# transferia/transferia

Hardware: AMD Instinct MI355X
Metric: ChangeItems/sec through CSV parse -> mask(ClientIP)+filter(EventDate) -> devnull, ClickBench hits, HBM-resident input (the PCIe-inclusive rate is `pcie_inclusive`) (higher is better)
Workload: dtype u8; 1 GPU; ClickBench hits-1M CSV parse -> mask(ip)+filter(EventDate) -> devnull (BASELINE.json configs[1]); columns=105, parallelism=row-range shard x1, no collective, rows_per_pass=1048576, csv_bytes_per_pass=838371857

## Files before the change

### transferia_amd/csrc/tf_common.hpp

```cpp
#pragma once
#include <hip/hip_runtime.h>

#include <cstdint>
#include <cstdio>
#include <cstring>
#include <memory>
#include <mutex>
#include <unordered_map>
#include <stdexcept>
#include <string>
#include <vector>

#include "../../include/tfgpu.h"

#ifndef TF_DYNAMIC_LDS
#define TF_DYNAMIC_LDS(type, name) extern __shared__ type name[]
#endif

#ifndef TF_GLOBAL_PTR
#define TF_GLOBAL_PTR(T, p) ((T *)(__attribute__((address_space(1))) T *)(p))
#endif

#ifndef TF_LOAD16_STREAM
__device__ __forceinline__ uint4 tf_load16_stream(const void *p) {
// ... 122 lines not shown
struct PinScope { PinScope() {} };
void d2h(void *dst, const void *src, size_t n);
void d2d(void *dst, const void *src, size_t n);
void sync();

inline bool repr_is_var(int r) { return r == TFGPU_R_STRING || r == TFGPU_R_BYTES || r == TFGPU_R_JSONNUM || r == TFGPU_R_JSON; }
inline size_t repr_width(int r) {
  switch (r) {
    case TFGPU_R_INT8: case TFGPU_R_UINT8: case TFGPU_R_BOOL: return 1;
    case TFGPU_R_INT16: case TFGPU_R_UINT16: return 2;
    case TFGPU_R_INT32: case TFGPU_R_UINT32: case TFGPU_R_FLOAT32: return 4;
    case TFGPU_R_INT64: case TFGPU_R_UINT64: case TFGPU_R_FLOAT64: case TFGPU_R_TIME: case TFGPU_R_DURATION: return 8;
    default: return 0;
  }
}

struct TextView {
  Buf src;
  Buf fstart;
  uint8_t quote = '"';
  bool jsonnum = false;
  bool has_special = true;
  Buf packed;
};
struct DColumn {
  std::string name;
  int dtype = TFGPU_T_INVALID;
  int repr = TFGPU_R_INVALID;
  Buf values, offsets, data, nanos, validity;
  Buf absent;
  uint64_t data_len = 0;
  std::shared_ptr<TextView> view;
  const Buf &payload() const { return (!data && view) ? view->packed : data; }
  bool lazy() const { return !data && view && !view->packed; }
};
void materialize(const struct ::tfgpu_dbatch &b, const std::vector<const DColumn *> *only = nullptr);
void dense(const struct ::tfgpu_dbatch *b, bool absent_ok = false);
void dense_locked(const struct ::tfgpu_dbatch &b);
int lanes_created();
uint64_t lane_generation();
std::unique_ptr<struct ::tfgpu_dbatch> snapshot(const struct ::tfgpu_dbatch &b);
bool has_absent(const struct ::tfgpu_dbatch &b);
Buf validity_minus_absent(const Buf &validity, const Buf &absent, int64_t nrows);
Buf find_device_block(const void *p);
void register_device_block(const Buf &b);

}

namespace tf {
struct PendingRows {
  std::shared_ptr<const struct ::tfgpu_dbatch> src;
  Buf sel;
};
}

struct tfgpu_dbatch {
  int64_t nrows = 0;
  std::vector<tf::DColumn> cols;
  std::shared_ptr<tf::PendingRows> pending;
// ... 4 lines not shown
  std::vector<std::pair<std::string, int>> schema;
  std::vector<std::string> key_names;
  std::vector<tf::DColumn> old_keys;
  tf::Buf old_present;
  std::string ns, table;
  tf::Buf kind, src_row, part_id;
  tf::Buf col_order;
};

struct tfgpu_dbuf {
  tf::Buf mem;
  uint64_t size = 0;
};

namespace tf {
inline std::unique_ptr<tfgpu_dbatch> shallow_copy(const tfgpu_dbatch &in) { return std::make_unique<tfgpu_dbatch>(in); }
template <class F> void materialize_where(const tfgpu_dbatch &b, F pred) {
  std::vector<const DColumn *> need;
  for (auto &c : b.cols) if (pred(c)) need.push_back(&c);
  materialize(b, &need);
}
void exclusive_scan_u32(const uint32_t *in, uint32_t *out, int64_t n, bool with_total);
void exclusive_scan_u32_segments(uint32_t *inout, int64_t seg_len, int nseg, int64_t seg_stride);
bool select_kept_u32(const uint32_t *keep, int64_t n, int32_t *sel, uint32_t *count);
const uint32_t *any_nonzero_to_host(const uint32_t *v, int64_t n);
const uint32_t *segment_totals_to_host(const uint32_t *scanned, int64_t seg_len, int nseg, int64_t seg_stride);
void sum_u32_segments_u64(const uint32_t *in, int64_t seg_len, int nseg, int64_t seg_stride, unsigned long long *totals);

}
```

### transferia_amd/csrc/tf_csv.hip

```cpp
#include <algorithm>
#include <cmath>
#include <cstdio>
#include <type_traits>

#include "tf_devfmt.hpp"
#include "tf_devparse.hpp"
#include "tf_devfloat.hpp"
#include "tf_segcopy.hpp"
#include "tf_textview.hpp"
#include "tf_wave.hpp"
#include "tf_swar.hpp"
#include "tf_gotime.hpp"
#include "tf_f64range.hpp"
#include "tf_plan.hpp"
#include "tf_strictcell.hpp"

#ifdef TF_CSV_ABLATE_BUILD
#define CSV_ABL(x) ((x).ablate)
#else
#define CSV_ABL(x) 0
#endif
namespace tf {

std::unique_ptr<tfgpu_dbatch> compact_rows(const tfgpu_dbatch &in, Buf keep);
// ... 1657 lines not shown

__global__ void csv_collect(const uint32_t *nerr, const uint32_t *last, const uint32_t *lens_all, int64_t seg_stride, int64_t nrows, int nstr, const uint32_t *fstart_all,
                            int64_t fstride, uint32_t *out, const uint32_t *spec, int64_t ntiles, int64_t skip, const uint32_t *lines_total, const uint32_t *ovf) {
  int i = threadIdx.x;
  if (ovf) {
    const uint32_t nl = *lines_total;
    if (i == 2) { out[2 + 2 * nstr] = nl; out[3 + 2 * nstr] = *ovf; }
    nrows = min(nrows, max((int64_t)nl - skip, (int64_t)0));
    if (i == 1) out[1] = *last;
  } else if (spec) {
    const uint32_t nl = ntiles ? (spec[2 + ntiles - 1] & SP_VAL) : 0u;
    if (i == 2) { out[2 + 2 * nstr] = nl; out[3 + 2 * nstr] = spec[1]; }
    nrows = min(nrows, max((int64_t)nl - skip, (int64_t)0));
    uint32_t le = 0;
    for (int64_t hi = ntiles - 1; hi >= 0 && le == 0; hi -= 64) {
      const int64_t t = hi - i;
      const uint32_t v = t >= 0 ? spec[2 + ntiles + t] : 0u;
      const uint64_t has = __ballot(v != 0);
      if (has) le = (uint32_t)__shfl((int)v, __ffsll((long long)has) - 1, 64);
    }
    if (i == 1) out[1] = le;
  } else if (i == 1) out[1] = *last;
  if (i == 0) out[0] = *nerr;
  for (int s = i; s < nstr; s += blockDim.x) { out[2 + s] = lens_all[(int64_t)s * seg_stride + nrows]; out[2 + nstr + s] = fstart_all[(int64_t)s * fstride + FS_HDR - 1]; }
}
__global__ void csv_zero_flags(uint32_t *fstart_all, int64_t fstride, int nstr, uint32_t *slow, uint32_t *gen, uint32_t *nerr, uint32_t *ovf) {
  for (int s = threadIdx.x; s < nstr; s += blockDim.x) fstart_all[(int64_t)s * fstride + FS_HDR - 1] = 0;
  if (threadIdx.x < 2) { slow[threadIdx.x] = 0; gen[threadIdx.x] = 0; }
  if (threadIdx.x == 2) *nerr = 0;
  if (threadIdx.x == 3 && ovf) *ovf = 0;
}
__global__ void csv_keep_from_err(const uint8_t *err, int64_t n, uint32_t *keep) {
  int64_t r = (int64_t)blockIdx.x * blockDim.x + threadIdx.x;
  if (r < n) keep[r] = err[r] ? 0u : 1u;
}

__global__ void csv_shift_rows(const uint32_t *row_start, int64_t n, uint32_t *out) {
  int64_t i = (int64_t)blockIdx.x * blockDim.x + threadIdx.x;
  if (i <= n) out[i] = row_start[i];
}

__global__ void __launch_bounds__(256) csv_ml_line_fn(const uint8_t *data, const uint32_t *row_start, int64_t nlines, uint8_t quote, uint8_t escape, uint8_t *fn) {
  const int64_t i = (int64_t)blockIdx.x * blockDim.x + threadIdx.x;
  if (i >= nlines) return;
  const uint64_t a = row_start[i], b = row_start[i + 1];
  if (b - a <= 1) { fn[i] = 2u | 4u; return; }
  MemBytes m(data);
// ... 86 lines not shown

uint32_t newline_starts(const uint8_t *data, uint64_t len, Buf *out) {
  hipStream_t st = ctx().stream;
  const int64_t ntiles = (int64_t)((len + NL_TILE - 1) / NL_TILE), ngran = (int64_t)((len + CSV_GRAN - 1) / CSV_GRAN);
  uint32_t n = 0;
  Buf tile_counts = dalloc((size_t)(ngran + 1) * 4);
  if (ntiles) {
    { KernelTimer t("csv_count_newlines"); csv_count_newlines<<<(unsigned)ntiles, NL_THREADS, 0, st>>>(data, len, ptr<uint32_t>(tile_counts), ngran); }
    exclusive_scan_u32(ptr<uint32_t>(tile_counts), ptr<uint32_t>(tile_counts), ngran, true);
    const uint32_t *h = d2h_u32(ptr<uint32_t>(tile_counts) + ngran);
    tf::sync();
    n = *h;
  }
  *out = dalloc_zero((size_t)(n + 2) * 4);
  if (n) { KernelTimer t("csv_line_index"); csv_line_index<<<(unsigned)ntiles, NL_THREADS, 0, st>>>(data, len, ptr<uint32_t>(tile_counts), ptr<uint32_t>(*out)); }
  return n;
}

static void materialize_cols(const tfgpu_dbatch &b, const std::vector<const DColumn *> *only, const uint8_t *text) {
  hipStream_t st = ctx().stream;
  const int64_t nrows = b.nrows;
  struct Grp { const uint8_t *src; uint8_t quote; std::vector<CopyCol> all, lng, sht; };
  std::vector<Grp> groups;
  auto visit = [&](const DColumn &d) {
    if (!d.lazy()) return;
    if (only && std::find(only->begin(), only->end(), &d) == only->end()) return;
    TextView &v = *d.view;
    const uint8_t *src = text ? text : ptr<uint8_t>(v.src);
    if (!src) throw Error(TFGPU_ERR_INVALID, "internal: text column " + d.name + " lost its source text");
    v.packed = dalloc(d.data_len + 8);
    CopyCol c{ptr<uint32_t>(d.offsets), ptr<uint32_t>(v.fstart), ptr<uint8_t>(v.packed), v.jsonnum ? 1 : 0, nullptr, 0};
    Grp *g = nullptr;
    for (auto &x : groups) if (x.src == src && x.quote == v.quote) g = &x;
    if (!g) { groups.push_back(Grp{src, v.quote, {}, {}, {}}); g = &groups.back(); }
    if (v.has_special) g->all.push_back(c);
    ((d.data_len >= (uint64_t)nrows * 8) ? g->lng : g->sht).push_back(c);
  };
  for (auto &d : b.cols) visit(d);
  for (auto &d : b.old_keys) visit(d);
  if (!nrows) return;
  for (auto &g : groups) {
    Buf ball = upload_small(g.all.data(), g.all.size() * sizeof(CopyCol));
    Buf blng = upload_small(g.lng.data(), g.lng.size() * sizeof(CopyCol)), bsht = upload_small(g.sht.data(), g.sht.size() * sizeof(CopyCol));
    KernelTimer t("csv_copy_words");
    if (!g.lng.empty()) { CopyParams cp{g.src, nrows, ptr<CopyCol>(blng), (int32_t)g.lng.size(), g.quote}; csv_copy_words<1><<<dim3((unsigned)((nrows + 255) / 256), (unsigned)g.lng.size()), 256, 0, st>>>(cp); }
    if (!g.sht.empty()) { CopyParams cp{g.src, nrows, ptr<CopyCol>(bsht), (int32_t)g.sht.size(), g.quote}; csv_copy_cells<<<dim3((unsigned)((nrows + 255) / 256), (unsigned)((g.sht.size() + CC_GROUP - 1) / CC_GROUP)), 256, 0, st>>>(cp); }
// ... 432 lines not shown
  if (ablate) {
    TF_HIP(hipMemsetAsync(lens_all->p, 0, (size_t)std::max(nstr, 1) * (size_t)seg_stride * 4, st));
    TF_HIP(hipMemsetAsync(fstart_all->p, 0, (size_t)std::max(nstr, 1) * (size_t)fstride * 4, st));
    TF_HIP(hipMemsetAsync(err->p, 0, (size_t)nrows + 16, st));
    for (auto &d : db->cols) { if (d.values) TF_HIP(hipMemsetAsync(d.values->p, 0, d.values->bytes, st)); if (d.nanos) TF_HIP(hipMemsetAsync(d.nanos->p, 0, d.nanos->bytes, st)); }
  }
  if (nrows && rowpath) {
    KernelTimer t("csv_parse_rows");
    csv_parse_rows<<<blocks_for(nrows, 256), 256, 0, st>>>(pp);
  } else if (nlines) {
    if (use_lanes) {
      const int64_t per_xcd = (ltiles + 7) / 8;
      KernelTimer t("csv_parse_lanes");
      csv_parse_lanes<<<(unsigned)(per_xcd * 8), CL_THREADS, 0, st>>>(pp);
    } else {
      const int64_t per_xcd = (rtiles + 7) / 8;
      KernelTimer t("csv_parse_regular");
      if (pp.col_lanes) csv_parse_cols<<<(unsigned)(spec ? rtiles : per_xcd * 8), CT_THREADS, 0, st>>>(pp);
      else csv_parse_regular<<<(unsigned)(spec ? rtiles : per_xcd * 8), CT_THREADS, 0, st>>>(pp);
    }
    { KernelTimer t("csv_parse_tiles_general"); csv_parse_tiles_general<<<(unsigned)std::min<int64_t>(ntiles + rtiles, 2048), CT_THREADS, 0, st>>>(pp); }
    { KernelTimer t("csv_parse_listed"); csv_parse_listed<<<(unsigned)std::min<int64_t>(blocks_for(slow_cap, 64), 1024), 64, 0, st>>>(pp); }
  }
  if (nrows && nstr) {
    csv_zero_err_lens<<<blocks_for(nrows, 256), 256, 0, st>>>(ptr<uint8_t>(err), nrows, ptr<CsvCol>(bcols), ncols, ahead ? ptr<uint32_t>(tile_counts) + ngran : nullptr, skip);
    exclusive_scan_u32_segments(ptr<uint32_t>(lens_all), nrows, nstr, seg_stride);
  } else if (nstr) {
    TF_HIP(hipMemsetAsync(lens_all->p, 0, (size_t)nstr * (size_t)seg_stride * 4, st));
  }
  Buf summary = dalloc((size_t)(2 * nstr + 4) * 4);
  csv_collect<<<1, 64, 0, st>>>(ptr<uint32_t>(nerr), rowpath ? ptr<uint32_t>(row_start) + nlines : pp.last_end, ptr<uint32_t>(lens_all),
                                seg_stride, nrows, nstr, ptr<uint32_t>(fstart_all), fstride, ptr<uint32_t>(summary), pp.spec, rtiles, skip,
                                ptr<uint32_t>(tile_counts) + (spec ? 0 : ngran), pp.ovf);
  const uint32_t *hsum = d2h_u32(summary->p, (size_t)(2 * nstr) + 4);
  tf::sync();
  const uint32_t hnerr = hsum[0], last = hsum[1];
  if (spec || ahead) {
    const uint32_t nl_true = hsum[2 + 2 * nstr], overflow = hsum[3 + 2 * nstr];
    if (overflow || nl_true > cap_lines || (int64_t)nl_true < skip || (nl_true && !last)) { *retry = true; return TFGPU_OK; }
    nlines = nl_true; nlogical = nl_true; nrows = (int64_t)nl_true - skip;
    db->nrows = nrows;
  }
  if (!rowpath && nlines >= 16 && last) { cx.csv_hint_bpl = (double)last / (double)nlines; cx.csv_hint_ncols = schema->ncols; }
  if (phases && !rowpath) {
    unsigned long long ph[8]; d2h(ph, bphase->p, sizeof ph); tf::sync();
    std::fprintf(stderr, "tfgpu csv phases (s_memtime ticks per workgroup, %lld tiles): stage %.0f classify %.0f fields %.0f index %.0f cells(wave 0) %.0f cells-barrier %.0f epilogue %.0f\n", (long long)rtiles,
                 (double)ph[0] / rtiles, (double)ph[1] / rtiles, (double)ph[2] / rtiles, (double)ph[3] / rtiles, (double)ph[4] / rtiles, (double)ph[5] / rtiles, (double)ph[6] / rtiles);
  }
  static const bool debug = [] { const char *e = std::getenv("TFGPU_CSV_DEBUG"); return e && e[0] == '1'; }();
  if (debug && !rowpath) {
    uint32_t g = 0, sl = 0;
    d2h(&g, gen->p, 4); d2h(&sl, slow->p, 4);
    tf::sync();
    std::fprintf(stderr, "tfgpu csv: %s, %lld tiles of %u KiB, %u general pieces; %u lines, %u per-row\n", use_lanes ? "lanes" : "regular", (long long)(use_lanes ? ltiles : rtiles), (use_lanes ? cl_tile(pp.tile_cpt) : tile_bytes) / 1024u, g, nlines, sl);
  }

  Buf src_block = staged ? staged : find_device_block(data);
  static const bool force_eager = [] { const char *e = std::getenv("TFGPU_CSV_EAGER"); return e && e[0] == '1'; }();
  for (int s = 0; s < nstr; s++) {
    DColumn &d = db->cols[(size_t)str_col_index[(size_t)s]];
    d.data_len = hsum[2 + s];
    d.offsets = subbuf(lens_all, (size_t)s * (size_t)seg_stride * 4, (size_t)(nrows + 1) * 4);
    if (rowpath) continue;
    auto v = std::make_shared<TextView>();
    v->src = src_block ? src_block : nullptr;
    v->fstart = subbuf(fstart_all, ((size_t)s * (size_t)fstride + FS_HDR) * 4, (size_t)std::max<int64_t>(nrows, 1) * 4);
    v->has_special = hsum[2 + nstr + s] != 0;
    v->quote = opts->quote_char; v->jsonnum = d.repr == TFGPU_R_JSONNUM;
    d.view = std::move(v);
  }
  if (nstr && rowpath) {
    std::vector<CopyCol> cc;
    for (int s = 0; s < nstr; s++) {
      DColumn &d = db->cols[(size_t)str_col_index[(size_t)s]];
      d.data = dalloc(d.data_len + 8);
      const CsvCol &hc = cols[(size_t)str_col_index[(size_t)s]];
      cc.push_back(CopyCol{ptr<uint32_t>(d.offsets), hc.fstart, ptr<uint8_t>(d.data), d.repr == TFGPU_R_JSONNUM ? 1 : 0, hc.patch, dp.empty() ? 0u : (uint32_t)dp.size()});
    }
    Buf bcc = up(cc.data(), cc.size() * sizeof(CopyCol));
    if (nrows) {
      CopyParams cp{data, nrows, ptr<CopyCol>(bcc), nstr, opts->quote_char};
      KernelTimer t("csv_copy_strings");
      csv_copy_strings<<<blocks_for(nrows, 256), 256, 0, st>>>(cp);
    }
  } else if (nstr && (!src_block || force_eager)) {
    materialize_from(*db, data);
  }

  for (int i : sys_cols) {
    std::string detail;
    const int rc = fill_system_column(db->cols[(size_t)i], nrows, opts->file_name, opts->row_number_base, nullptr, opts->hide_system_cols, &detail);
// ... 40 lines not shown
```

### transferia_amd/csrc/tf_devcol.hpp

```cpp
#pragma once
#include "tf_common.hpp"

namespace tf {

struct DCol {
  const void *values;
  const uint32_t *offsets;
  const uint8_t *data;
  const int32_t *nanos;
  const uint8_t *validity;
  int32_t repr;
  int32_t dtype;
};
static inline DCol dcol_of(const DColumn &c) {
  DCol d;
  d.values = c.values ? c.values->p : nullptr;
  d.offsets = ptr<uint32_t>(c.offsets);
  if (c.lazy()) throw Error(TFGPU_ERR_INVALID, "internal: text column " + c.name + " read before materialize()");
  d.data = ptr<uint8_t>(c.payload());
  d.nanos = ptr<int32_t>(c.nanos);
  d.validity = ptr<uint8_t>(c.validity);
  d.repr = c.repr; d.dtype = c.dtype;
  return d;
}
__device__ __forceinline__ bool is_valid(const DCol &c, int64_t r) { return !c.validity || ((c.validity[r >> 3] >> (r & 7)) & 1); }


}
```

### transferia_amd/csrc/tf_mask.hip

```cpp
#include "tf_plan.hpp"
#include "tf_rows.hpp"
#include "tf_devrow.hpp"
#include "tf_emit.hpp"

namespace tf {
__constant__ uint32_t SHA_K[64] = {
    0x428a2f98, 0x71374491, 0xb5c0fbcf, 0xe9b5dba5, 0x3956c25b, 0x59f111f1, 0x923f82a4, 0xab1c5ed5, 0xd807aa98, 0x12835b01, 0x243185be,
    0x550c7dc3, 0x72be5d74, 0x80deb1fe, 0x9bdc06a7, 0xc19bf174, 0xe49b69c1, 0xefbe4786, 0x0fc19dc6, 0x240ca1cc, 0x2de92c6f, 0x4a7484aa,
    0x5cb0a9dc, 0x76f988da, 0x983e5152, 0xa831c66d, 0xb00327c8, 0xbf597fc7, 0xc6e00bf3, 0xd5a79147, 0x06ca6351, 0x14292967, 0x27b70a85,
    0x2e1b2138, 0x4d2c6dfc, 0x53380d13, 0x650a7354, 0x766a0abb, 0x81c2c92e, 0x92722c85, 0xa2bfe8a1, 0xa81a664b, 0xc24b8b70, 0xc76c51a3,
    0xd192e819, 0xd6990624, 0xf40e3585, 0x106aa070, 0x19a4c116, 0x1e376c08, 0x2748774c, 0x34b0bcb5, 0x391c0cb3, 0x4ed8aa4a, 0x5b9cca4f,
    0x682e6ff3, 0x748f82ee, 0x78a5636f, 0x84c87814, 0x8cc70208, 0x90befffa, 0xa4506ceb, 0xbef9a3f7, 0xc67178f2};

__device__ __forceinline__ uint32_t rotr32(uint32_t x, int n) { return __builtin_rotateright32(x, n); }

__device__ __forceinline__ void sha256_compress(uint32_t st[8], uint32_t w[16]) {
  uint32_t a = st[0], b = st[1], c = st[2], d = st[3], e = st[4], f = st[5], g = st[6], h = st[7];
#pragma unroll
  for (int i = 0; i < 64; i++) {
    if (i >= 16) {
      uint32_t w15 = w[(i - 15) & 15], w2 = w[(i - 2) & 15];
      uint32_t s0 = rotr32(w15, 7) ^ rotr32(w15, 18) ^ (w15 >> 3);
      uint32_t s1 = rotr32(w2, 17) ^ rotr32(w2, 19) ^ (w2 >> 10);
      w[i & 15] = w[i & 15] + s0 + w[(i - 7) & 15] + s1;
// ... 101 lines not shown
      uint32_t n0 = (half >> 12) & 15, n1 = (half >> 8) & 15, n2 = (half >> 4) & 15, n3 = half & 15;
      auto hx = [](uint32_t n) { return n + (n < 10 ? '0' : 'a' - 10); };
      o[k] = hx(n0) | hx(n1) << 8 | hx(n2) << 16 | hx(n3) << 24;
    }
    dst[q] = make_uint4(o[0], o[1], o[2], o[3]);
  }
  p.offsets[ro] = (uint32_t)(ro * 64);
  if (ro == p.nrows - 1) p.offsets[p.nrows] = (uint32_t)(p.nrows * 64);
}


void mask_precheck(const tfgpu_plan &p, const tfgpu_dbatch &in) {
  for (auto &c : (in.pending ? in.pending->src->cols : in.cols)) {
    if (!p.mask_has(c.name)) continue;
    bool done = false;
    for (auto &r : in.replaced) if (r.name == c.name) done = true;
    if (done) continue;
    require_serializable(c, "mask_field");
    if ((uint64_t)in.nrows * 64 > 0xFFFFFFFFull) throw Error(TFGPU_ERR_UNSUPPORTED, "mask_field: batch too large for 32-bit offsets; split the batch by rows");
  }
}

std::unique_ptr<tfgpu_dbatch> apply_mask(const tfgpu_plan &p, const tfgpu_dbatch &in) {
  auto out = shallow_copy(in);
  for (auto &sc : out->schema) if (p.mask_has(sc.first)) sc.second = TFGPU_T_UTF8;
  hipStream_t st = ctx().stream;
  const tfgpu_dbatch &from = in.pending ? *in.pending->src : in;
  const int32_t *sel = in.pending ? ptr<int32_t>(in.pending->sel) : nullptr;
  auto replaced_at = [&](const std::string &name) -> int { for (size_t i = 0; i < in.replaced.size(); i++) if (in.replaced[i].name == name) return (int)i; return -1; };
  materialize_where(from, [&](const DColumn &c) { return p.mask_has(c.name) && replaced_at(c.name) < 0; });
  const int64_t n = in.nrows;
  auto mask_one = [&](const DColumn &c, const int32_t *through) {
    require_serializable(c, "mask_field");
    if ((uint64_t)n * 64 > 0xFFFFFFFFull) throw Error(TFGPU_ERR_UNSUPPORTED, "mask_field: batch too large for 32-bit offsets; split the batch by rows");
    DColumn o;
    o.name = c.name; o.dtype = TFGPU_T_UTF8; o.repr = TFGPU_R_STRING;
    o.data_len = (uint64_t)n * 64;
    o.data = dalloc(o.data_len);
    o.offsets = dalloc((size_t)(n + 1) * 4);
    MaskParams mp;
    mp.col = dcol_of(c);
    std::memcpy(mp.ipad, p.ipad_state, sizeof mp.ipad);
    std::memcpy(mp.opad, p.opad_state, sizeof mp.opad);
    mp.nrows = n; mp.out = ptr<uint8_t>(o.data); mp.offsets = ptr<uint32_t>(o.offsets); mp.sel = through;
    {
      KernelTimer t("mask_hmac_sha256", n);
      if (n) mask_hmac_kernel<<<grid_for(n, 256), 256, 0, st>>>(mp);
    }
    if (!n) TF_HIP(hipMemsetAsync(o.offsets->p, 0, 4, st));
    return o;
  };
  if (!in.pending) {
    for (auto &c : out->cols) if (p.mask_has(c.name)) {
// ... 16 lines not shown
```

### transferia_amd/csrc/tf_rows.hip

```cpp
#include <chrono>
#include <thread>

#include "tf_rows.hpp"
#include "tf_devrow.hpp"
#include "tf_segcopy.hpp"
#include "tf_textview.hpp"

namespace tf {
__global__ void __launch_bounds__(256) build_selection_kernel(const uint32_t *__restrict__ keep_scan, int64_t n, int32_t *__restrict__ sel) {
  int64_t i = (int64_t)blockIdx.x * blockDim.x + threadIdx.x;
  if (i >= n) return;
  uint32_t a = keep_scan[i], b = keep_scan[i + 1];
  if (a != b) sel[a] = (int32_t)i;
}

struct GFix { const void *in; void *out; int32_t width; int32_t pad; };
template <class T> __device__ __forceinline__ void gather_run(const GFix *__restrict__ a, int lo, int hi, int32_t s, int64_t k) {
  constexpr int U = 8;
  int i = lo;
  for (; i + U <= hi; i += U) {
    T v[U];
#pragma unroll
    for (int q = 0; q < U; q++) v[q] = TF_GLOBAL_PTR(const T, a[i + q].in)[s];
#pragma unroll
// ... 73 lines not shown
    if (n) { fsv = g.fstart[sel[k]]; if (cell_plain(fsv)) n = 0; }
  }
  text_copy_special_wave(g.in_data, g.quote, g.out_data, g.jsonnum != 0, fsv, o0, n, threadIdx.x & 63);
}
__global__ void collect_totals(const uint32_t *lens_all, int64_t seg_stride, int64_t m, int nv, uint32_t *out) {
  for (int s = threadIdx.x; s < nv; s += blockDim.x) out[s] = lens_all[(int64_t)s * seg_stride + m];
}

static std::unique_ptr<tfgpu_dbatch> gather_batch(const tfgpu_dbatch &in, const Buf &sel, int64_t m, const std::vector<DColumn> *skip = nullptr) {
  if (in.col_order) throw Error(TFGPU_ERR_UNSUPPORTED, "the batch's rows carry their own ColumnNames order (tfgpu_batch.col_order: a collapsed TOAST batch); row-moving steps do not carry it — "
                                                       "view / download, the native queue format and the Debezium emitter read it");
  auto out = std::make_unique<tfgpu_dbatch>();
  out->nrows = m; out->ns = in.ns; out->table = in.table; out->schema = in.schema;
  hipStream_t st = ctx().stream;
  const int32_t *sp = ptr<int32_t>(sel);
  unsigned g = grid_for(m, 256);
  KernelTimer t("compact_gather");
  static const bool eager_text = [] { const char *e = std::getenv("TFGPU_CSV_EAGER"); return e && e[0] == '1'; }();
  std::vector<GFix> fx; std::vector<GVar> vr; std::vector<size_t> var_cols; std::vector<GBit> bits;
  const size_t ncur = in.cols.size(), nall = ncur + in.old_keys.size();
  auto col_at = [&](size_t i) -> const DColumn & { return i < ncur ? in.cols[i] : in.old_keys[i - ncur]; };
  out->cols.reserve(ncur); out->old_keys.reserve(in.old_keys.size());
  out->key_names = in.key_names;
  int nvar = 0;
  for (size_t i = 0; i < nall; i++) if (repr_is_var(col_at(i).repr) && !(skip && i < ncur && [&] { for (auto &r : *skip) if (r.name == in.cols[i].name) return true; return false; }())) nvar++;
  const int64_t seg_stride = ((m + 1 + 3) / 4) * 4;
  Buf lens_all = nvar ? dalloc((size_t)nvar * (size_t)seg_stride * 4 + 16) : nullptr;
  auto skipped = [&](size_t ai) -> const DColumn * {
    if (!skip || ai >= ncur) return nullptr;
    for (auto &r : *skip) if (r.name == in.cols[ai].name) return &r;
    return nullptr;
  };
  for (size_t ai = 0; ai < nall; ai++) {
    const DColumn &c = col_at(ai);
    if (const DColumn *have = skipped(ai)) { out->cols.push_back(*have); continue; }
    DColumn o;
    o.name = c.name; o.dtype = c.dtype; o.repr = c.repr;
    if (repr_is_var(c.repr)) {
      size_t si = vr.size();
      o.offsets = subbuf(lens_all, si * (size_t)seg_stride * 4, (size_t)(m + 1) * 4);
      if (!c.lazy() || eager_text) o.data = dalloc(c.data_len + 8);
      o.data_len = c.data_len;
      if (c.lazy() && !eager_text) {
        if (!c.view->src) throw Error(TFGPU_ERR_INVALID, "internal: text column " + c.name + " lost its source text");
        auto v = std::make_shared<TextView>();
        v->src = c.view->src; v->fstart = dalloc((size_t)std::max<int64_t>(m, 1) * 4);
        v->has_special = c.view->has_special; v->quote = c.view->quote; v->jsonnum = c.view->jsonnum;
        fx.push_back(GFix{c.view->fstart->p, v->fstart->p, 4, 0});
        o.view = std::move(v);
        o.data = nullptr;
        vr.push_back(GVar{ptr<uint32_t>(c.offsets), nullptr, ptr<uint32_t>(o.offsets), nullptr, nullptr, 0, 0, 0});
      } else if (c.lazy()) {
        if (!c.view->src) throw Error(TFGPU_ERR_INVALID, "internal: text column " + c.name + " lost its source text");
        vr.push_back(GVar{ptr<uint32_t>(c.offsets), ptr<uint8_t>(c.view->src), ptr<uint32_t>(o.offsets), ptr<uint8_t>(o.data), ptr<uint32_t>(c.view->fstart), c.view->quote, c.view->jsonnum ? 1u : 0u, c.view->has_special ? 1u : 0u});
      } else vr.push_back(GVar{ptr<uint32_t>(c.offsets), ptr<uint8_t>(c.payload()), ptr<uint32_t>(o.offsets), ptr<uint8_t>(o.data), nullptr, 0, 0, 0});
      var_cols.push_back(ai);
    } else {
      size_t w = repr_width(c.repr);
      o.values = dalloc((size_t)m * w);
      fx.push_back(GFix{c.values->p, o.values->p, (int32_t)w, 0});
      if (c.nanos) { o.nanos = dalloc((size_t)m * 4); fx.push_back(GFix{c.nanos->p, o.nanos->p, 4, 0}); }
// ... 27 lines not shown
    exclusive_scan_u32_segments(ptr<uint32_t>(lens_all), m, nvar, seg_stride);
    if (m) {
      std::vector<GVar> lng, sht;
      for (size_t i = 0; i < vr.size(); i++) if (vr[i].out_data) ((col_at(var_cols[i]).data_len >= (uint64_t)in.nrows * 8) ? lng : sht).push_back(vr[i]);
      Buf blng = upload_const(lng.data(), lng.size() * sizeof(GVar)), bsht = upload_const(sht.data(), sht.size() * sizeof(GVar));
      if (!lng.empty()) gather_bytes_all<1><<<dim3(grid_for(m, 256), (unsigned)lng.size()), 256, 0, st>>>(ptr<GVar>(blng), sp, m);
      if (!sht.empty()) gather_bytes_cells<<<dim3(grid_for(m, 256), (unsigned)sht.size()), 256, 0, st>>>(ptr<GVar>(bsht), sp, m);
      std::vector<GVar> lz;
      for (auto &x : vr) if (x.fstart && x.has_special) lz.push_back(x);
      if (!lz.empty()) {
        Buf blz = upload_const(lz.data(), lz.size() * sizeof(GVar));
        gather_text_special<<<dim3(grid_for(m, 256), (unsigned)lz.size()), 256, 0, st>>>(ptr<GVar>(blz), sp, m);
      }
    }
    Buf tot = dalloc((size_t)nvar * 4);
    collect_totals<<<1, 64, 0, st>>>(ptr<uint32_t>(lens_all), seg_stride, m, nvar, ptr<uint32_t>(tot));
    const uint32_t *h = d2h_u32(tot->p, (size_t)nvar);
    sync();
    for (int i = 0; i < nvar; i++) out_at(var_cols[(size_t)i]).data_len = h[i];
  }
  return out;
}

std::unique_ptr<tfgpu_dbatch> gather_rows(const tfgpu_dbatch &in, const Buf &sel, int64_t m) { return gather_batch(in, sel, m); }

static bool lazy_rows_on() {
  static const bool off = [] { const char *e = std::getenv("TFGPU_LAZY_ROWS"); return e && e[0] == '0'; }();
  return !off;
}
std::unique_ptr<tfgpu_dbatch> compact(const tfgpu_dbatch &in, Buf keep , bool lazy) {
  int64_t n = in.nrows;
  Buf sel = dalloc((size_t)n * 4 + 4);
  const uint32_t *hm;
  if (select_kept_u32(ptr<uint32_t>(keep), n, ptr<int32_t>(sel), ptr<uint32_t>(keep) + n)) hm = d2h_u32(ptr<uint32_t>(keep) + n);
  else {
    exclusive_scan_u32(ptr<uint32_t>(keep), ptr<uint32_t>(keep), n, true);
    hm = d2h_u32(ptr<uint32_t>(keep) + n);
    if (n) build_selection_kernel<<<grid_for(n, 256), 256, 0, ctx().stream>>>(ptr<uint32_t>(keep), n, ptr<int32_t>(sel));
  }
  sync();
  const uint32_t m = *hm;
  if ((int64_t)m == n) return shallow_copy(in);
  if (lazy && lazy_rows_on() && !in.pending && m) {
    auto out = std::make_unique<tfgpu_dbatch>();
    out->nrows = m; out->ns = in.ns; out->table = in.table; out->schema = in.schema; out->key_names = in.key_names;
    auto pr = std::make_shared<PendingRows>();
// ... 96 lines not shown
```

### transferia_amd/csrc/tf_scan.hip

```cpp
#include "tf_common.hpp"
#include "tf_wave.hpp"

namespace tf {

static constexpr int SCAN_THREADS = 256;
static constexpr int SCAN_WAVES = SCAN_THREADS / 64;
static constexpr int SCAN_ITEMS = 16;
static constexpr int SCAN_TILE = SCAN_THREADS * SCAN_ITEMS;
static constexpr int64_t RAW_SUMS_MAX = 1024;

__device__ __forceinline__ void scan_load16(const uint32_t *__restrict__ src, int64_t base, int64_t n, bool fast, uint32_t v[SCAN_ITEMS]) {
  if (fast) {
    const uint4 *p = reinterpret_cast<const uint4 *>(src + base);
#pragma unroll
    for (int i = 0; i < SCAN_ITEMS / 4; i++) { uint4 q = p[i]; v[4 * i] = q.x; v[4 * i + 1] = q.y; v[4 * i + 2] = q.z; v[4 * i + 3] = q.w; }
  } else {
#pragma unroll
    for (int i = 0; i < SCAN_ITEMS; i++) v[i] = (base + i < n) ? src[base + i] : 0;
  }
}

__global__ void __launch_bounds__(SCAN_THREADS) scan_reduce_kernel(const uint32_t *__restrict__ in, uint32_t *__restrict__ sums,
                                                                  int64_t n, int64_t seg_stride, int64_t nblocks) {
  __shared__ uint32_t lds[SCAN_WAVES];
// ... 121 lines not shown
}

__global__ void __launch_bounds__(256) any_nonzero_kernel(const uint32_t *v, int64_t n, uint32_t *flag) {
  bool hit = false;
  for (int64_t i = (int64_t)blockIdx.x * 256 + threadIdx.x; i < n; i += (int64_t)gridDim.x * 256) hit |= v[i] != 0;
  if (__ballot(hit) && (threadIdx.x & 63) == 0) atomicOr(flag, 1u);
}
const uint32_t *any_nonzero_to_host(const uint32_t *v, int64_t n) {
  Buf flag = dalloc_zero(4);
  if (n > 0) any_nonzero_kernel<<<(unsigned)std::min<int64_t>((n + 255) / 256, 1024), 256, 0, ctx().stream>>>(v, n, ptr<uint32_t>(flag));
  return d2h_u32(flag->p, 1);
}

void exclusive_scan_u32(const uint32_t *in, uint32_t *out, int64_t n, bool with_total) {
  KernelTimer t("scan_u32");
  scan_impl(in, out, n, 0, 1, with_total);
}

void exclusive_scan_u32_segments(uint32_t *inout, int64_t seg_len, int nseg, int64_t seg_stride) {
  if (nseg <= 0) return;
  KernelTimer t("scan_u32_segments");
  scan_impl(inout, inout, seg_len, seg_stride, nseg, true);
}

}
```

### transferia_amd/csrc/tf_sizeof.hip

```cpp
#include "tf_devcol.hpp"
#include "tf_wave.hpp"

using namespace tf;

namespace {

constexpr int SZ_MAXCOLS = 1024;
constexpr int SZ_DEPTH = 64;

struct SzCol {
  const uint32_t *offsets;
  const uint8_t *data;
  const uint8_t *validity;
  const uint8_t *absent;
  uint32_t fixed;
  uint32_t var;
};

__device__ inline int hexval(uint8_t c) { return c <= '9' ? c - '0' : (c | 0x20) - 'a' + 10; }

__device__ uint64_t json_deepsize(const uint8_t *p, uint32_t n, bool float_numbers, bool *overflow) {
  uint64_t size = 0;
  uint64_t is_obj = 0;
  uint64_t want_key = 0;
// ... 37 lines not shown
    else if (c == 'n') { i += 4; v = 0; }
    else {
      uint32_t s = i;
      while (i < n && p[i] != ',' && p[i] != '}' && p[i] != ']' && p[i] != ' ' && p[i] != '\t' && p[i] != '\n' && p[i] != '\r') i++;
      v = float_numbers ? 8 : 16 + (uint64_t)(i - s);
    }
    if (key) { size += v; want_key &= ~(1ull << (depth - 1)); }
    else size += (depth ? 16 : 0) + v;
  }
  return size;
}

__global__ void __launch_bounds__(256) deepsizeof_rows(const SzCol *cols, int ncols, int64_t n, uint32_t flags, uint64_t *per_row, unsigned long long *total, uint32_t *deep) {
  int64_t r = (int64_t)blockIdx.x * blockDim.x + threadIdx.x;
  uint64_t s = 0;
  if (r < n) {
    s = 24 + 16ull * (uint64_t)ncols;
    for (int c = 0; c < ncols; c++) {
      const SzCol k = cols[c];
      if (k.absent && ((k.absent[r >> 3] >> (r & 7)) & 1)) { s -= 16; continue; }
      if (k.validity && !((k.validity[r >> 3] >> (r & 7)) & 1)) continue;
      s += k.fixed;
      if (k.var == 1) s += k.offsets[r + 1] - k.offsets[r];
      else if (k.var == 2) {
        bool over = false;
        s += json_deepsize(k.data + k.offsets[r], k.offsets[r + 1] - k.offsets[r], flags & 1u, &over);
        if (over) atomicAdd(deep, 1u);
      }
    }
    if (per_row) per_row[r] = s;
  }
  uint64_t w = s;
  for (int o = 32; o > 0; o >>= 1) w += __shfl_down(w, o, 64);
  if ((threadIdx.x & 63) == 0 && w) atomicAdd(total, (unsigned long long)w);
}

}

#define TF_API_BEGIN try {
#define TF_API_END                                                        \
  }                                                                       \
  catch (const tf::Error &e) { return tf::fail(e.code, e.what()); }       \
  catch (const std::bad_alloc &) { return tf::fail(TFGPU_ERR_NOMEM, "out of host memory"); } \
  catch (const std::exception &e) { return tf::fail(TFGPU_ERR_INVALID, e.what()); }

extern "C" int tfgpu_dbatch_deepsizeof(const tfgpu_dbatch *in, uint32_t flags, uint64_t *per_row, uint64_t *total) {
// ... 10 lines not shown
  std::vector<SzCol> h((size_t)std::max(ncols, 1));
  {
    std::vector<const DColumn *> need;
    for (auto &c : in->cols) if (c.repr == TFGPU_R_JSON) need.push_back(&c);
    if (!need.empty()) materialize(*in, &need);
  }
  for (int c = 0; c < ncols; c++) {
    const DColumn &d = in->cols[(size_t)c];
    SzCol &k = h[(size_t)c];
    k.offsets = ptr<uint32_t>(d.offsets);
    k.data = nullptr;
    k.validity = ptr<uint8_t>(d.validity);
    k.absent = ptr<uint8_t>(d.absent);
    k.var = 0;
    switch (d.repr) {
      case TFGPU_R_STRING: case TFGPU_R_JSONNUM: k.fixed = 16; k.var = 1; break;
      case TFGPU_R_BYTES: k.fixed = 24; k.var = 1; break;
      case TFGPU_R_JSON: k.fixed = 0; k.var = 2; k.data = ptr<uint8_t>(d.payload()); break;
      case TFGPU_R_TIME: k.fixed = 24; break;
      default:
        k.fixed = (uint32_t)repr_width(d.repr);
        if (!k.fixed) return tf::fail(TFGPU_ERR_UNSUPPORTED, "tfgpu_dbatch_deepsizeof: column " + d.name + " has no Go value form");
    }
  }
  KernelTimer t("deepsizeof_rows");
  Buf dcols = upload_small(h.data(), h.size() * sizeof(SzCol));
  Buf acc = dalloc_zero(16);
  Buf rows = per_row ? dalloc((size_t)n * 8) : Buf();
  deepsizeof_rows<<<(unsigned)((n + 255) / 256), 256, 0, cx.stream>>>(ptr<SzCol>(dcols), ncols, n, flags, ptr<uint64_t>(rows), ptr<unsigned long long>(acc),
                                                                   ptr<uint32_t>(acc) + 2);
  uint64_t back[2];
  d2h(back, ptr<uint8_t>(acc), 16);
  if (per_row) d2h(per_row, ptr<uint8_t>(rows), (size_t)n * 8);
  sync();
  if ((uint32_t)back[1]) return tf::fail(TFGPU_ERR_UNSUPPORTED, "tfgpu_dbatch_deepsizeof: an `any` value nests deeper than 64 containers");
  *total = back[0];
  return TFGPU_OK;
  TF_API_END
}
```

### transferia_amd/csrc/tf_transform.hip

```cpp
#include "tf_plan.hpp"
#include "tf_rows.hpp"
#include "tf_devrow.hpp"

namespace tf {

std::vector<int> chain_sequence(const tfgpu_plan *const *plans, int n, std::vector<std::vector<int>> *hopped) {
  static const bool off = [] { const char *e = std::getenv("TFGPU_CHAIN_REORDER"); return e && e[0] == '0'; }();
  std::vector<int> seq((size_t)n);
  for (int i = 0; i < n; i++) seq[(size_t)i] = i;
  if (hopped) hopped->assign((size_t)n, {});
  if (off) return seq;
  for (int j = 1; j < n; j++) {
    if (plans[seq[(size_t)j]]->kind != PK_FILTER_ROWS) continue;
    const tfgpu_plan &f = *plans[seq[(size_t)j]];
    int k = j;
    std::vector<int> over;
    while (k > 0 && plans[seq[(size_t)k - 1]]->kind == PK_MASK) {
      const tfgpu_plan &m = *plans[seq[(size_t)k - 1]];
      bool reads = false;
      for (auto &e : f.exprs) for (auto &t : e.terms) if (m.mask_has(t.attr)) reads = true;
      if (reads) break;
      over.insert(over.begin(), seq[(size_t)k - 1]);
      std::swap(seq[(size_t)k - 1], seq[(size_t)k]);
      k--;
// ... 233 lines not shown
        for (size_t i = 0; i < in.cols.size(); i++) if (in.cols[i].name == t.attr) { d.col = (int32_t)i; break; }
        d.op = t.op; d.vtype = t.vtype; d.is_list = t.is_list;
        switch (t.vtype) {
          case FV_FLOAT: d.nvals = (int32_t)t.floats.size(); d.ioff = (int32_t)floats.size(); floats.insert(floats.end(), t.floats.begin(), t.floats.end()); break;
          case FV_STRING:
            d.nvals = (int32_t)t.strs.size(); d.soff = (int32_t)soff.size();
            for (auto &s : t.strs) { soff.push_back((uint32_t)sdata.size()); sdata += s; }
            soff.push_back((uint32_t)sdata.size());
            break;
          default: d.nvals = (int32_t)t.ints.size(); d.ioff = (int32_t)ints.size(); ints.insert(ints.end(), t.ints.begin(), t.ints.end());
        }
        terms.push_back(d);
      }
      expr_start.push_back((int32_t)terms.size());
    }
  }
  {
    std::vector<const DColumn *> need;
    for (auto &t : terms) if (t.col >= 0) need.push_back(&in.cols[(size_t)t.col]);
    materialize(in, &need);
  }
  std::vector<DCol> cols;
  for (auto &c : in.cols) {
    if (c.lazy()) { DColumn shell = c; shell.view = nullptr; cols.push_back(dcol_of(shell)); }
    else cols.push_back(dcol_of(c));
  }
  auto up = [&](const void *src, size_t bytes) { return upload_const(src, bytes); };
  Buf bcols = up(cols.data(), cols.size() * sizeof(DCol)), bterms = up(terms.data(), terms.size() * sizeof(DTerm));
  Buf bexpr = up(expr_start.data(), expr_start.size() * 4), bints = up(ints.data(), ints.size() * 8), bfl = up(floats.data(), floats.size() * 8);
  Buf bsoff = up(soff.data(), soff.size() * 4), bsd = up(sdata.data(), sdata.size());
  Buf keep = dalloc((size_t)(n + 1) * 4), err = dalloc((size_t)n + 1), eterm = dalloc((size_t)n * 4 + 4), nerr = dalloc_zero(4);
  FilterParams fp;
  fp.cols = ptr<DCol>(bcols); fp.ncols = (int32_t)cols.size(); fp.terms = ptr<DTerm>(bterms); fp.expr_start = ptr<int32_t>(bexpr);
  fp.nexpr = table_applies ? (int32_t)p_exprs.size() : 0;
  fp.ints = ptr<int64_t>(bints); fp.floats = ptr<double>(bfl); fp.str_off = ptr<uint32_t>(bsoff); fp.str_data = ptr<uint8_t>(bsd);
  fp.absent = nullptr;
  Buf babs;
  {
    std::vector<const uint8_t *> abs;
    bool any = false;
    for (auto &c : in.cols) { abs.push_back(ptr<uint8_t>(c.absent)); any = any || c.absent; }
    if (any) { babs = up(abs.data(), abs.size() * sizeof(const uint8_t *)); fp.absent = reinterpret_cast<const uint8_t *const *>(babs->p); }
  }
  fp.kind = check_kinds ? ptr<uint8_t>(in.kind) : nullptr; fp.nrows = n; fp.keep = ptr<uint32_t>(keep); fp.err = ptr<uint8_t>(err); fp.err_term = ptr<int32_t>(eterm); fp.nerr = ptr<uint32_t>(nerr);
  if (!table_applies) fp.nexpr = -1;
  {
    KernelTimer t("filter_rows_eval");
// ... 360 lines not shown
```

Before: 963.2 million rows/s.

## Defer CSV string-length prefix scan until offsets are actually needed

The CSV parser no longer zeroes error lengths or runs the segmented exclusive scan over every string column's lengths. Each lazy text view now keeps raw per-row lengths, and offsets are computed on demand by ensure_text_offsets when a column is materialized or gathered eagerly. Row gathers carry the lengths along instead of scanning them, and deepsizeof reads the lengths directly. This removes a scan over roughly a hundred columns per pass when most columns are never materialized. The cost is added complexity, a global mutex, a host sync inside ensure_text_offsets, and a new lens_only state that every consumer must handle.

New measurement: 1.036 billion rows/s (median of 6 runs). +7.6%, better.

```diff
diff --git a/transferia_amd/csrc/tf_common.hpp b/transferia_amd/csrc/tf_common.hpp
--- a/transferia_amd/csrc/tf_common.hpp
+++ b/transferia_amd/csrc/tf_common.hpp
@@ -168,6 +168,9 @@
   bool jsonnum = false;
   bool has_special = true;
   Buf packed;
+  Buf lens;
+  Buf offsets;
+  uint64_t total = 0;
 };
 struct DColumn {
   std::string name;
@@ -179,8 +182,10 @@
   std::shared_ptr<TextView> view;
   const Buf &payload() const { return (!data && view) ? view->packed : data; }
   bool lazy() const { return !data && view && !view->packed; }
+  bool lens_only() const { return view && view->lens && !offsets; }
 };
 void materialize(const struct ::tfgpu_dbatch &b, const std::vector<const DColumn *> *only = nullptr);
+void ensure_text_offsets(const struct ::tfgpu_dbatch &b);
 void dense(const struct ::tfgpu_dbatch *b, bool absent_ok = false);
 void dense_locked(const struct ::tfgpu_dbatch &b);
 int lanes_created();
@@ -231,6 +236,7 @@
 }
 void exclusive_scan_u32(const uint32_t *in, uint32_t *out, int64_t n, bool with_total);
 void exclusive_scan_u32_segments(uint32_t *inout, int64_t seg_len, int nseg, int64_t seg_stride);
+void exclusive_scan_u32_segments(const uint32_t *in, uint32_t *out, int64_t seg_len, int nseg, int64_t seg_stride);
 bool select_kept_u32(const uint32_t *keep, int64_t n, int32_t *sel, uint32_t *count);
 const uint32_t *any_nonzero_to_host(const uint32_t *v, int64_t n);
 const uint32_t *segment_totals_to_host(const uint32_t *scanned, int64_t seg_len, int nseg, int64_t seg_stride);
diff --git a/transferia_amd/csrc/tf_csv.hip b/transferia_amd/csrc/tf_csv.hip
--- a/transferia_amd/csrc/tf_csv.hip
+++ b/transferia_amd/csrc/tf_csv.hip
@@ -1703,7 +1703,7 @@
     if (i == 1) out[1] = le;
   } else if (i == 1) out[1] = *last;
   if (i == 0) out[0] = *nerr;
-  for (int s = i; s < nstr; s += blockDim.x) { out[2 + s] = lens_all[(int64_t)s * seg_stride + nrows]; out[2 + nstr + s] = fstart_all[(int64_t)s * fstride + FS_HDR - 1]; }
+  for (int s = i; s < nstr; s += blockDim.x) { out[2 + s] = lens_all ? lens_all[(int64_t)s * seg_stride + nrows] : 0u; out[2 + nstr + s] = fstart_all[(int64_t)s * fstride + FS_HDR - 1]; }
 }
 __global__ void csv_zero_flags(uint32_t *fstart_all, int64_t fstride, int nstr, uint32_t *slow, uint32_t *gen, uint32_t *nerr, uint32_t *ovf) {
   for (int s = threadIdx.x; s < nstr; s += blockDim.x) fstart_all[(int64_t)s * fstride + FS_HDR - 1] = 0;
@@ -1836,6 +1836,13 @@
   const int64_t nrows = b.nrows;
   struct Grp { const uint8_t *src; uint8_t quote; std::vector<CopyCol> all, lng, sht; };
   std::vector<Grp> groups;
+  {
+    bool need = false;
+    auto look = [&](const DColumn &d) { if (d.lens_only() && !(only && std::find(only->begin(), only->end(), &d) == only->end())) need = true; };
+    for (auto &d : b.cols) look(d);
+    for (auto &d : b.old_keys) look(d);
+    if (need) ensure_text_offsets(b);
+  }
   auto visit = [&](const DColumn &d) {
     if (!d.lazy()) return;
     if (only && std::find(only->begin(), only->end(), &d) == only->end()) return;
@@ -2314,14 +2321,19 @@
     { KernelTimer t("csv_parse_tiles_general"); csv_parse_tiles_general<<<(unsigned)std::min<int64_t>(ntiles + rtiles, 2048), CT_THREADS, 0, st>>>(pp); }
     { KernelTimer t("csv_parse_listed"); csv_parse_listed<<<(unsigned)std::min<int64_t>(blocks_for(slow_cap, 64), 1024), 64, 0, st>>>(pp); }
   }
-  if (nrows && nstr) {
+  Buf src_block = staged ? staged : find_device_block(data);
+  static const bool force_eager = [] { const char *e = std::getenv("TFGPU_CSV_EAGER"); return e && e[0] == '1'; }();
+  static const bool scan_eager = [] { const char *e = std::getenv("TFGPU_CSV_SCAN_EAGER"); return e && e[0] == '1'; }();
+  const bool lens_state = !rowpath && src_block && !force_eager && !scan_eager;
+  if (lens_state) {
+  } else if (nrows && nstr) {
     csv_zero_err_lens<<<blocks_for(nrows, 256), 256, 0, st>>>(ptr<uint8_t>(err), nrows, ptr<CsvCol>(bcols), ncols, ahead ? ptr<uint32_t>(tile_counts) + ngran : nullptr, skip);
     exclusive_scan_u32_segments(ptr<uint32_t>(lens_all), nrows, nstr, seg_stride);
   } else if (nstr) {
     TF_HIP(hipMemsetAsync(lens_all->p, 0, (size_t)nstr * (size_t)seg_stride * 4, st));
   }
   Buf summary = dalloc((size_t)(2 * nstr + 4) * 4);
-  csv_collect<<<1, 64, 0, st>>>(ptr<uint32_t>(nerr), rowpath ? ptr<uint32_t>(row_start) + nlines : pp.last_end, ptr<uint32_t>(lens_all),
+  csv_collect<<<1, 64, 0, st>>>(ptr<uint32_t>(nerr), rowpath ? ptr<uint32_t>(row_start) + nlines : pp.last_end, lens_state ? nullptr : ptr<uint32_t>(lens_all),
                                 seg_stride, nrows, nstr, ptr<uint32_t>(fstart_all), fstride, ptr<uint32_t>(summary), pp.spec, rtiles, skip,
                                 ptr<uint32_t>(tile_counts) + (spec ? 0 : ngran), pp.ovf);
   const uint32_t *hsum = d2h_u32(summary->p, (size_t)(2 * nstr) + 4);
@@ -2347,18 +2359,19 @@
     std::fprintf(stderr, "tfgpu csv: %s, %lld tiles of %u KiB, %u general pieces; %u lines, %u per-row\n", use_lanes ? "lanes" : "regular", (long long)(use_lanes ? ltiles : rtiles), (use_lanes ? cl_tile(pp.tile_cpt) : tile_bytes) / 1024u, g, nlines, sl);
   }
 
-  Buf src_block = staged ? staged : find_device_block(data);
-  static const bool force_eager = [] { const char *e = std::getenv("TFGPU_CSV_EAGER"); return e && e[0] == '1'; }();
   for (int s = 0; s < nstr; s++) {
     DColumn &d = db->cols[(size_t)str_col_index[(size_t)s]];
-    d.data_len = hsum[2 + s];
-    d.offsets = subbuf(lens_all, (size_t)s * (size_t)seg_stride * 4, (size_t)(nrows + 1) * 4);
+    if (!lens_state) {
+      d.data_len = hsum[2 + s];
+      d.offsets = subbuf(lens_all, (size_t)s * (size_t)seg_stride * 4, (size_t)(nrows + 1) * 4);
+    }
     if (rowpath) continue;
     auto v = std::make_shared<TextView>();
     v->src = src_block ? src_block : nullptr;
     v->fstart = subbuf(fstart_all, ((size_t)s * (size_t)fstride + FS_HDR) * 4, (size_t)std::max<int64_t>(nrows, 1) * 4);
     v->has_special = hsum[2 + nstr + s] != 0;
     v->quote = opts->quote_char; v->jsonnum = d.repr == TFGPU_R_JSONNUM;
+    if (lens_state) v->lens = subbuf(lens_all, (size_t)s * (size_t)seg_stride * 4, (size_t)nrows * 4);
     d.view = std::move(v);
   }
   if (nstr && rowpath) {
diff --git a/transferia_amd/csrc/tf_devcol.hpp b/transferia_amd/csrc/tf_devcol.hpp
--- a/transferia_amd/csrc/tf_devcol.hpp
+++ b/transferia_amd/csrc/tf_devcol.hpp
@@ -16,7 +16,7 @@
   DCol d;
   d.values = c.values ? c.values->p : nullptr;
   d.offsets = ptr<uint32_t>(c.offsets);
-  if (c.lazy()) throw Error(TFGPU_ERR_INVALID, "internal: text column " + c.name + " read before materialize()");
+  if (c.lazy() || c.lens_only()) throw Error(TFGPU_ERR_INVALID, "internal: text column " + c.name + " read before materialize()");
   d.data = ptr<uint8_t>(c.payload());
   d.nanos = ptr<int32_t>(c.nanos);
   d.validity = ptr<uint8_t>(c.validity);
diff --git a/transferia_amd/csrc/tf_mask.hip b/transferia_amd/csrc/tf_mask.hip
--- a/transferia_amd/csrc/tf_mask.hip
+++ b/transferia_amd/csrc/tf_mask.hip
@@ -147,13 +147,13 @@
 }
 
 std::unique_ptr<tfgpu_dbatch> apply_mask(const tfgpu_plan &p, const tfgpu_dbatch &in) {
-  auto out = shallow_copy(in);
-  for (auto &sc : out->schema) if (p.mask_has(sc.first)) sc.second = TFGPU_T_UTF8;
   hipStream_t st = ctx().stream;
   const tfgpu_dbatch &from = in.pending ? *in.pending->src : in;
   const int32_t *sel = in.pending ? ptr<int32_t>(in.pending->sel) : nullptr;
   auto replaced_at = [&](const std::string &name) -> int { for (size_t i = 0; i < in.replaced.size(); i++) if (in.replaced[i].name == name) return (int)i; return -1; };
   materialize_where(from, [&](const DColumn &c) { return p.mask_has(c.name) && replaced_at(c.name) < 0; });
+  auto out = shallow_copy(in);
+  for (auto &sc : out->schema) if (p.mask_has(sc.first)) sc.second = TFGPU_T_UTF8;
   const int64_t n = in.nrows;
   auto mask_one = [&](const DColumn &c, const int32_t *through) {
     require_serializable(c, "mask_field");
diff --git a/transferia_amd/csrc/tf_rows.hip b/transferia_amd/csrc/tf_rows.hip
--- a/transferia_amd/csrc/tf_rows.hip
+++ b/transferia_amd/csrc/tf_rows.hip
@@ -119,10 +119,18 @@
   auto col_at = [&](size_t i) -> const DColumn & { return i < ncur ? in.cols[i] : in.old_keys[i - ncur]; };
   out->cols.reserve(ncur); out->old_keys.reserve(in.old_keys.size());
   out->key_names = in.key_names;
-  int nvar = 0;
-  for (size_t i = 0; i < nall; i++) if (repr_is_var(col_at(i).repr) && !(skip && i < ncur && [&] { for (auto &r : *skip) if (r.name == in.cols[i].name) return true; return false; }())) nvar++;
+  {
+    bool need = false;
+    for (size_t i = 0; i < nall; i++) if (col_at(i).lens_only() && (eager_text || !col_at(i).lazy())) need = true;
+    if (need) ensure_text_offsets(in);
+  }
+  auto stays_lens = [&](const DColumn &c) { return c.lens_only() && c.lazy() && !eager_text; };
+  int nvar = 0, nlens = 0;
+  for (size_t i = 0; i < nall; i++) if (repr_is_var(col_at(i).repr) && !(skip && i < ncur && [&] { for (auto &r : *skip) if (r.name == in.cols[i].name) return true; return false; }())) (stays_lens(col_at(i)) ? nlens : nvar)++;
   const int64_t seg_stride = ((m + 1 + 3) / 4) * 4;
   Buf lens_all = nvar ? dalloc((size_t)nvar * (size_t)seg_stride * 4 + 16) : nullptr;
+  Buf lens_kept = nlens ? dalloc((size_t)nlens * (size_t)seg_stride * 4 + 16) : nullptr;
+  size_t li = 0;
   auto skipped = [&](size_t ai) -> const DColumn * {
     if (!skip || ai >= ncur) return nullptr;
     for (auto &r : *skip) if (r.name == in.cols[ai].name) return &r;
@@ -133,7 +141,17 @@
     if (const DColumn *have = skipped(ai)) { out->cols.push_back(*have); continue; }
     DColumn o;
     o.name = c.name; o.dtype = c.dtype; o.repr = c.repr;
-    if (repr_is_var(c.repr)) {
+    if (repr_is_var(c.repr) && stays_lens(c)) {
+      if (!c.view->src) throw Error(TFGPU_ERR_INVALID, "internal: text column " + c.name + " lost its source text");
+      auto v = std::make_shared<TextView>();
+      v->src = c.view->src; v->fstart = dalloc((size_t)std::max<int64_t>(m, 1) * 4);
+      v->has_special = c.view->has_special; v->quote = c.view->quote; v->jsonnum = c.view->jsonnum;
+      v->lens = subbuf(lens_kept, li++ * (size_t)seg_stride * 4, (size_t)m * 4);
+      fx.push_back(GFix{c.view->fstart->p, v->fstart->p, 4, 0});
+      fx.push_back(GFix{c.view->lens->p, v->lens->p, 4, 0});
+      o.view = std::move(v);
+    } else if (repr_is_var(c.repr)) {
+      if (c.lens_only()) throw Error(TFGPU_ERR_INVALID, "internal: text column " + c.name + " gathered before its lengths were scanned");
       size_t si = vr.size();
       o.offsets = subbuf(lens_all, si * (size_t)seg_stride * 4, (size_t)(m + 1) * 4);
       if (!c.lazy() || eager_text) o.data = dalloc(c.data_len + 8);
@@ -207,6 +225,55 @@
   return out;
 }
 
+static std::mutex g_text_mu;
+void ensure_text_offsets(const tfgpu_dbatch &b) {
+  std::vector<DColumn *> cols;
+  for (auto &c : b.cols) if (c.lens_only()) cols.push_back(const_cast<DColumn *>(&c));
+  for (auto &c : b.old_keys) if (c.lens_only()) cols.push_back(const_cast<DColumn *>(&c));
+  if (cols.empty()) return;
+  std::lock_guard<std::mutex> tl(g_text_mu);
+  const int64_t n = b.nrows;
+  std::vector<TextView *> todo;
+  for (auto *c : cols) {
+    TextView *v = c->view.get();
+    if ((int64_t)(v->lens->bytes / 4) != n) throw Error(TFGPU_ERR_INVALID, "internal: text column " + c->name + " holds lengths of another row count");
+    if (!v->offsets && std::find(todo.begin(), todo.end(), v) == todo.end()) todo.push_back(v);
+  }
+  if (!todo.empty() && n == 0) {
+    for (auto *v : todo) { v->total = 0; v->offsets = dalloc_zero(16); }
+  } else if (!todo.empty()) {
+    std::sort(todo.begin(), todo.end(), [](const TextView *x, const TextView *y) { return x->lens->p < y->lens->p; });
+    struct Run { size_t first; int nseg; int64_t stride; Buf out; const uint32_t *tot; };
+    std::vector<Run> runs;
+    const int64_t own_stride = ((n + 1 + 3) / 4) * 4;
+    for (size_t i = 0; i < todo.size();) {
+      Run r{i, 1, own_stride, nullptr, nullptr};
+      if (i + 1 < todo.size()) {
+        const int64_t d = ptr<uint32_t>(todo[i + 1]->lens) - ptr<uint32_t>(todo[i]->lens);
+        if (d >= n + 1 && d % 4 == 0 && d <= 2 * own_stride + 64) {
+          r.stride = d;
+          while (r.first + (size_t)r.nseg < todo.size() && ptr<uint32_t>(todo[r.first + (size_t)r.nseg]->lens) - ptr<uint32_t>(todo[r.first + (size_t)r.nseg - 1]->lens) == d) r.nseg++;
+        }
+      }
+      i += (size_t)r.nseg;
+      runs.push_back(r);
+    }
+    for (auto &r : runs) {
+      r.out = dalloc((size_t)r.nseg * (size_t)r.stride * 4 + 16);
+      exclusive_scan_u32_segments(ptr<uint32_t>(todo[r.first]->lens), ptr<uint32_t>(r.out), n, r.nseg, r.stride);
+      r.tot = segment_totals_to_host(ptr<uint32_t>(r.out), n, r.nseg, r.stride);
+    }
+    sync();
+    for (auto &r : runs)
+      for (int s = 0; s < r.nseg; s++) {
+        TextView *v = todo[r.first + (size_t)s];
+        v->total = r.tot[s];
+        v->offsets = subbuf(r.out, (size_t)s * (size_t)r.stride * 4, (size_t)(n + 1) * 4);
+      }
+  }
+  for (auto *c : cols) { c->data_len = c->view->total; c->offsets = c->view->offsets; }
+}
+
 std::unique_ptr<tfgpu_dbatch> gather_rows(const tfgpu_dbatch &in, const Buf &sel, int64_t m) { return gather_batch(in, sel, m); }
 
 static bool lazy_rows_on() {
diff --git a/transferia_amd/csrc/tf_scan.hip b/transferia_amd/csrc/tf_scan.hip
--- a/transferia_amd/csrc/tf_scan.hip
+++ b/transferia_amd/csrc/tf_scan.hip
@@ -167,5 +167,10 @@
   KernelTimer t("scan_u32_segments");
   scan_impl(inout, inout, seg_len, seg_stride, nseg, true);
 }
+void exclusive_scan_u32_segments(const uint32_t *in, uint32_t *out, int64_t seg_len, int nseg, int64_t seg_stride) {
+  if (nseg <= 0) return;
+  KernelTimer t("scan_u32_segments");
+  scan_impl(in, out, seg_len, seg_stride, nseg, true);
+}
 
 }
diff --git a/transferia_amd/csrc/tf_sizeof.hip b/transferia_amd/csrc/tf_sizeof.hip
--- a/transferia_amd/csrc/tf_sizeof.hip
+++ b/transferia_amd/csrc/tf_sizeof.hip
@@ -83,6 +83,7 @@
       if (k.validity && !((k.validity[r >> 3] >> (r & 7)) & 1)) continue;
       s += k.fixed;
       if (k.var == 1) s += k.offsets[r + 1] - k.offsets[r];
+      else if (k.var == 3) s += k.offsets[r];
       else if (k.var == 2) {
         bool over = false;
         s += json_deepsize(k.data + k.offsets[r], k.offsets[r + 1] - k.offsets[r], flags & 1u, &over);
@@ -139,6 +140,7 @@
         k.fixed = (uint32_t)repr_width(d.repr);
         if (!k.fixed) return tf::fail(TFGPU_ERR_UNSUPPORTED, "tfgpu_dbatch_deepsizeof: column " + d.name + " has no Go value form");
     }
+    if (k.var == 1 && d.lens_only()) { k.var = 3; k.offsets = ptr<uint32_t>(d.view->lens); }
   }
   KernelTimer t("deepsizeof_rows");
   Buf dcols = upload_small(h.data(), h.size() * sizeof(SzCol));
diff --git a/transferia_amd/csrc/tf_transform.hip b/transferia_amd/csrc/tf_transform.hip
--- a/transferia_amd/csrc/tf_transform.hip
+++ b/transferia_amd/csrc/tf_transform.hip
@@ -279,7 +279,7 @@
   }
   std::vector<DCol> cols;
   for (auto &c : in.cols) {
-    if (c.lazy()) { DColumn shell = c; shell.view = nullptr; cols.push_back(dcol_of(shell)); }
+    if (c.lazy() || c.lens_only()) { DColumn shell = c; shell.view = nullptr; cols.push_back(dcol_of(shell)); }
     else cols.push_back(dcol_of(c));
   }
   auto up = [&](const void *src, size_t bytes) { return upload_const(src, bytes); };
```
